# rusty-fast-solvers/rusty-compression

Hardware: AMD Instinct MI355X
Metric: GB/s + compressions/sec, 8192x8192 f64 rank-128 rSVD+ID (higher is better)
Workload: dtype f64

## Files before the change

rusty_compression_amd/csrc/kernels_qr.hip:

```cpp
#include "rc_common.hpp"
#include "rc_device.hpp"

namespace rc {

static __host__ __device__ inline int64_t cdiv(int64_t a, int64_t b) { return (a + b - 1) / b; }

template <typename T> struct Num;
template <> struct Num<double> {
    static __host__ __device__ inline double tol3z() { return 1.0536712127723509e-08; }
};
template <> struct Num<float> {
    static __host__ __device__ inline float tol3z() { return 2.44140625e-04f; }
};

template <typename T>
__device__ inline T wsum(T v) {
#pragma unroll
    for (int off = 32; off > 0; off >>= 1) v += __shfl_xor(v, off, 64);
    return v;
}

template <typename T, int TPC>
__device__ inline T group_sum(T v, T *sh ) {
    v = wsum(v);
// ... 258 lines not shown
        const int64_t rem_cols = n - j - 1;
        if (rem_cols <= 0) continue;
        const int64_t rem = m - j;
        const int64_t c64 = cdiv(rem, 64), c256 = cdiv(rem, 256);
#define RC_APPLY(TPC, MAXE)                                                                                       \
    hipLaunchKernelGGL((k_qr_apply<T, TPC, MAXE>), dim3((unsigned)cdiv(rem_cols, 256 / TPC)), dim3(256), 0,      \
                       c->stream, w, j, pv, jpvt, vn1, vn2, tau)
        if (c64 <= 2 && rem_cols >= 2048) {
            constexpr int CPW = 4;
            hipLaunchKernelGGL((k_qr_apply_short<T, CPW>), dim3((unsigned)cdiv(rem_cols, 4 * CPW)), dim3(256), 0, c->stream, w, j, pv, jpvt, vn1, vn2, tau);
        }
        else if (c64 <= 2) RC_APPLY(64, 2);
        else if (c64 <= 8) RC_APPLY(64, 8);
        else if (c256 <= 8) RC_APPLY(256, 8);
        else if (c256 <= 16) RC_APPLY(256, 16);
        else if (c256 <= 32) RC_APPLY(256, 32);
        else
            hipLaunchKernelGGL(k_qr_apply_general<T>, dim3((unsigned)rem_cols), dim3(256), 0, c->stream, w, j, pv, jpvt, vn1, vn2, tau);
#undef RC_APPLY
    }
}

template <typename T>
__global__ __launch_bounds__(256) void k_extract_r(Mat<T> w, const int64_t *jpvt, Mat<T> r) {
    const bool col_fast = (r.cs <= r.rs);
    const int64_t total = r.rows * r.cols;
    for (int64_t e = blockIdx.x * (int64_t)blockDim.x + threadIdx.x; e < total; e += (int64_t)gridDim.x * blockDim.x) {
        int64_t i, p;
        if (col_fast) { i = e / r.cols; p = e - i * r.cols; }
        else { p = e / r.rows; i = e - p * r.rows; }
        r.at(i, p) = (i <= p) ? w.p[jpvt[p] * w.cs + i] : (T)0;
    }
}
template <typename T>
void extract_r(rc_context *c, Mat<T> w, const int64_t *jpvt, Mat<T> r) {
    if (r.empty()) return;
    int grid = (int)std::min<int64_t>(cdiv(r.rows * r.cols, 256), 8192);
    hipLaunchKernelGGL(k_extract_r<T>, dim3(grid), dim3(256), 0, c->stream, w, jpvt, r);
}

template <typename T, int MAXE>
__global__ __launch_bounds__(256) void k_form_q(Mat<T> w, const int64_t *jpvt, const T *tau, int64_t k, Mat<T> qw) {
    __shared__ T sh[4];
    const int64_t m = w.rows;
    const int64_t cq = blockIdx.x;
    const int tid = threadIdx.x;
    T x[MAXE];
#pragma unroll
    for (int e = 0; e < MAXE; ++e) {
        int64_t i = tid + (int64_t)e * 256;
        x[e] = (i == cq) ? (T)1 : (T)0;
    }
    for (int64_t j = (cq < k - 1 ? cq : k - 1); j >= 0; --j) {
        const T tj = tau[j];
        if (tj == (T)0) continue;
// ... 22 lines not shown
}
template <typename T>
__global__ __launch_bounds__(256) void k_form_q_general(Mat<T> w, const int64_t *jpvt, const T *tau, int64_t k, Mat<T> qw) {
    __shared__ T sh[4];
    const int64_t m = w.rows;
    const int64_t cq = blockIdx.x;
    const int tid = threadIdx.x;
    T *x = qw.p + cq * qw.cs;
    for (int64_t i = tid; i < m; i += 256) x[i] = (i == cq) ? (T)1 : (T)0;
    for (int64_t j = (cq < k - 1 ? cq : k - 1); j >= 0; --j) {
        const T tj = tau[j];
        if (tj == (T)0) continue;
        const T *vcol = w.p + jpvt[j] * w.cs;
        const int64_t i0 = tid >= j ? tid : tid + ((j - tid + 255) / 256) * 256;
        T dot = 0;
        for (int64_t i = i0; i < m; i += 256) dot += ((i == j) ? (T)1 : vcol[i]) * x[i];
        dot = group_sum<T, 256>(dot, sh);
        const T f = tj * dot;
        for (int64_t i = i0; i < m; i += 256) x[i] -= f * ((i == j) ? (T)1 : vcol[i]);
    }
}

template <typename T, int NE>
__global__ __launch_bounds__(1024) void k_form_q_small(Mat<T> w, const int64_t *jpvt, const T *tau, int k, Mat<T> qw) {
    extern __shared__ __attribute__((aligned(16))) char smem_raw[];
    T *V = reinterpret_cast<T *>(smem_raw);
    T *tl = V + (size_t)k * 8 * NE;
    const int m = (int)w.rows;
    constexpr int LD = 8 * NE;
    for (int e = threadIdx.x; e < k * LD; e += blockDim.x) {
        const int j = e / LD, i = e - j * LD;
        V[e] = (i < j || i >= m) ? (T)0 : (i == j) ? (T)1 : w.p[jpvt[j] * w.cs + i];
    }
    for (int j = threadIdx.x; j < k; j += blockDim.x) tl[j] = tau[j];
    __syncthreads();
    const int l8 = threadIdx.x & 7, cq = threadIdx.x >> 3;
    if (cq >= qw.cols) return;
    T x[NE];
#pragma unroll
    for (int e = 0; e < NE; ++e) x[e] = (l8 + 8 * e == cq) ? (T)1 : (T)0;
    for (int j = cq < k - 1 ? cq : k - 1; j >= 0; --j) {
        const T tj = tl[j];
        if (tj == (T)0) continue;
        const T *vj = V + (size_t)j * LD + l8;
        T v[NE];
        T dot = 0;
#pragma unroll
        for (int e = 0; e < NE; ++e) {
            v[e] = vj[8 * e];
            dot = fma(v[e], x[e], dot);
        }
        dot = group_sum_dpp<8>(dot);
        const T f = tj * dot;
#pragma unroll
        for (int e = 0; e < NE; ++e) x[e] = fma(-f, v[e], x[e]);
    }
    T *out = qw.p + (int64_t)cq * qw.cs;
#pragma unroll
    for (int e = 0; e < NE; ++e) {
        const int i = l8 + 8 * e;
        if (i < m) out[i] = x[e];
    }
}

template <typename T>
__global__ __launch_bounds__(256) void k_extract_v(Mat<T> w, const int64_t *jpvt, Mat<T> vm) {
    const int64_t j = blockIdx.y;
    const T *col = w.p + jpvt[j] * w.cs;
    T *out = vm.p + j * vm.cs;
    for (int64_t i = blockIdx.x * 256 + threadIdx.x; i < vm.rows; i += (int64_t)gridDim.x * 256)
        out[i] = (i < j) ? (T)0 : (i == j) ? (T)1 : col[i];
}
template <typename T>
__global__ __launch_bounds__(1024) void k_build_t(Mat<T> sgram, const T *tau, Mat<T> tm) {
    extern __shared__ __attribute__((aligned(16))) char smem_raw[];
    T *svec = reinterpret_cast<T *>(smem_raw);
    T *trow = svec + tm.rows;
    const int k = (int)tm.rows;
    const int ld = k | 1;
    const int tid = threadIdx.x;
    for (int e = tid; e < k * ld; e += 1024) trow[e] = 0;
    __syncthreads();
    for (int j = 0; j < k; ++j) {
        for (int l = tid; l < j; l += 1024) svec[l] = sgram.at(l, j);
        __syncthreads();
// ... 105 lines not shown
#pragma unroll
                        for (int i2 = 0; i2 < ii; ++i2) acc[i2] -= tile[i2][ii] * acc[ii];
                    }
                }
            }
        }
        if (active) {
#pragma unroll
            for (int ii = 0; ii < NB; ++ii)
                if (r0 + ii < k) b.at(r0 + ii, col) = acc[ii];
        }
    }
}
template <typename T>
void trsm_upper(rc_context *c, Mat<T> t, Mat<T> b) {
    RC_REQUIRE(t.rows == t.cols && t.rows == b.rows, RC_INVALID_ARGUMENT, "trsm: shape mismatch");
    if (b.empty()) return;
    ProfScope ps(c, "op:trsm_upper k=%lld nrhs=%lld", (long long)t.rows, (long long)b.cols);
    hipLaunchKernelGGL(k_trsm_upper<T>, dim3((unsigned)cdiv(b.cols, 256)), dim3(256), 0, c->stream, t, b);
}

template <bool CHECKED> struct IdzCheck {};
template <> struct IdzCheck<true> { const int64_t *inv; int *health; };
template <typename T, bool FROM_R, bool CHECKED = false>
__global__ __launch_bounds__(256) void k_id_z(Mat<T> w, const int64_t *jpvt, int64_t k, Mat<T> z, IdzCheck<CHECKED> chk = {}) {
    static_assert(FROM_R || !CHECKED, "the ?geqp3-format variant only ever sees a jpvt the library wrote");
    constexpr int NB = 16;
    __shared__ T tile[NB][NB + 1];
    const int64_t n = w.cols;
    const int64_t p = blockIdx.x * (int64_t)blockDim.x + threadIdx.x;
    bool owns = p < n;
    if constexpr (CHECKED) {
        if (owns && chk.inv[p] < 0) {
            for (int64_t i = 0; i < k; ++i) z.at(i, p) = (T)0;
            atomicOr(chk.health, 32);
        }
        const int64_t e = owns ? jpvt[p] : -1;
        owns = (uint64_t)e < (uint64_t)n && chk.inv[e] == p;
    }
    const bool inside = owns;
    const int64_t dc = inside ? jpvt[p] : 0;
    const bool active = inside && p >= k;
    const T *bcol = FROM_R ? w.p + (inside ? p : 0) * w.cs : w.p + dc * w.cs;
    const int64_t brs = FROM_R ? w.rs : 1;
    const int64_t nblk = (k + NB - 1) / NB;
    const int ti = threadIdx.x / NB, tj = threadIdx.x % NB;
    if (inside && p < k)
        for (int64_t i = 0; i < k; ++i) z.at(i, dc) = (i == p) ? (T)1 : (T)0;
    for (int64_t bi = nblk - 1; bi >= 0; --bi) {
        const int64_t r0 = bi * NB;
        T acc[NB];
#pragma unroll
        for (int ii = 0; ii < NB; ++ii) acc[ii] = (active && r0 + ii < k) ? bcol[(r0 + ii) * brs] : (T)0;
        for (int64_t bj = nblk - 1; bj >= bi; --bj) {
            const int64_t c0 = bj * NB;
            __syncthreads();
            {
                const int64_t i = r0 + ti, l = c0 + tj;
                tile[ti][tj] = (i < k && l < k && i <= l) ? (FROM_R ? w.at(i, l) : w.p[jpvt[l] * w.cs + i]) : (T)0;
            }
            __syncthreads();
            if (bj > bi) {
                T x[NB];
#pragma unroll
                for (int jj = 0; jj < NB; ++jj) x[jj] = (active && c0 + jj < k) ? z.at(c0 + jj, dc) : (T)0;
#pragma unroll
                for (int jj = 0; jj < NB; ++jj)
#pragma unroll
                    for (int ii = 0; ii < NB; ++ii) acc[ii] -= tile[ii][jj] * x[jj];
            } else {
#pragma unroll
                for (int ii = NB - 1; ii >= 0; --ii) {
                    if (r0 + ii < k) {
                        acc[ii] /= tile[ii][ii];
#pragma unroll
                        for (int i2 = 0; i2 < ii; ++i2) acc[i2] -= tile[i2][ii] * acc[ii];
                    }
                }
            }
        }
        if (active) {
#pragma unroll
            for (int ii = 0; ii < NB; ++ii)
                if (r0 + ii < k) z.at(r0 + ii, dc) = acc[ii];
        }
    }
}
template <typename T>
void column_id_from_qrcp(rc_context *c, Mat<T> a, Mat<T> w, int64_t k, const int64_t *jpvt, Mat<T> cm, Mat<T> z) {
    RC_REQUIRE(w.rs == 1 && a.rows == w.rows && a.cols == w.cols && cm.rows == a.rows && cm.cols == k && z.rows == k && z.cols == a.cols && k <= std::min(a.rows, a.cols),
               RC_INVALID_ARGUMENT, "column_id_from_qrcp: shape mismatch");
    if (a.cols == 0 || k == 0) return;
    ProfScope ps(c, "op:column_id_from_qrcp %lldx%lld k=%lld", (long long)a.rows, (long long)a.cols, (long long)k);
    hipLaunchKernelGGL((k_id_z<T, false>), dim3((unsigned)cdiv(a.cols, 256)), dim3(256), 0, c->stream, w, jpvt, k, z);
    gather_cols(c, a, jpvt, cm);
}
template <typename T>
void id_z_from_r(rc_context *c, Mat<T> r, int64_t k, const int64_t *ind, Mat<T> z) {
    RC_REQUIRE(r.rows == k && z.rows == k && z.cols == r.cols && k <= r.cols, RC_INVALID_ARGUMENT, "id_z_from_r: shape mismatch");
    if (r.cols == 0 || k == 0) return;
    ProfScope ps(c, "op:id_z_from_r k=%lld n=%lld", (long long)k, (long long)r.cols);
    hipLaunchKernelGGL((k_id_z<T, true>), dim3((unsigned)cdiv(r.cols, 256)), dim3(256), 0, c->stream, r, ind, k, z);
}
template <typename T>
void id_z_from_r_checked(rc_context *c, Mat<T> r, int64_t k, const int64_t *ind, const int64_t *inv, Mat<T> z) {
    RC_REQUIRE(r.rows == k && z.rows == k && z.cols == r.cols && k <= r.cols, RC_INVALID_ARGUMENT, "id_z_from_r: shape mismatch");
    if (r.cols == 0 || k == 0) return;
    ProfScope ps(c, "op:id_z_from_r_checked k=%lld n=%lld", (long long)k, (long long)r.cols);
    hipLaunchKernelGGL((k_id_z<T, true, true>), dim3((unsigned)cdiv(r.cols, 256)), dim3(256), 0, c->stream, r, ind, k, z, IdzCheck<true>{inv, c->health_word()});
}

#define RC_INST(T)                                                                                         \
    template void column_id_from_qrcp<T>(rc_context *, Mat<T>, Mat<T>, int64_t, const int64_t *, Mat<T>, Mat<T>); \
    template void id_z_from_r<T>(rc_context *, Mat<T>, int64_t, const int64_t *, Mat<T>);                 \
    template void id_z_from_r_checked<T>(rc_context *, Mat<T>, int64_t, const int64_t *, const int64_t *, Mat<T>); \
    template void geqp3_inplace<T>(rc_context *, Mat<T>, int64_t, bool, int64_t *, T *, T *);             \
    template void extract_r<T>(rc_context *, Mat<T>, const int64_t *, Mat<T>);                             \
    template void form_q<T>(rc_context *, Mat<T>, const int64_t *, const T *, int64_t, Mat<T>);           \
    template void trsm_upper<T>(rc_context *, Mat<T>, Mat<T>);
RC_INST(double)
RC_INST(float)
#undef RC_INST

}

namespace rc {

template <typename T>
__global__ __launch_bounds__(256) void k_wq_init(Mat<T> qacc, Mat<T> rphys) {
    const int64_t tq = qacc.rows * qacc.cols, tr = rphys.rows * rphys.cols;
    for (int64_t e = blockIdx.x * (int64_t)blockDim.x + threadIdx.x; e < tq + tr; e += (int64_t)gridDim.x * blockDim.x) {
        if (e < tq) { int64_t i = e % qacc.rows, c2 = e / qacc.rows; qacc.p[c2 * qacc.cs + i] = (i == c2) ? (T)1 : (T)0; }
        else rphys.p[e - tq] = 0;
    }
}

template <typename T>
__global__ __launch_bounds__(1024) void k_wq_pivot(Mat<T> b, Mat<T> qacc, Mat<T> rphys, int64_t j, int64_t *jpvt, T *vn1, T *vn2, T *tau) {
    extern __shared__ __attribute__((aligned(16))) char smem_raw[];
    const int m = (int)b.rows;
// ... 248 lines not shown
```

rusty_compression_amd/csrc/kernels_tsqr.hip:

```cpp
#include "rc_common.hpp"
#include "rc_device.hpp"

namespace rc {

static __host__ __device__ inline int64_t cdiv(int64_t a, int64_t b) { return (a + b - 1) / b; }

template <typename T> struct TNum;
template <> struct TNum<double> {
    static __device__ inline double tol3z() { return 1.0536712127723509e-08; }
    static __device__ inline double tiny() { return 1e-300; }
};
template <> struct TNum<float> {
    static __device__ inline float tol3z() { return 2.44140625e-04f; }
    static __device__ inline float tiny() { return 1e-30f; }
};

template <typename T>
__device__ inline T wave_sum64(T v) {
#pragma unroll
    for (int off = 32; off > 0; off >>= 1) v += __shfl_xor(v, off, 64);
    return v;
}
template <typename T>
__device__ inline T row_sum16(T v) {
// ... 257 lines not shown
                    vn1[p] = vn * fast_sqrt_pos(temp);
                }
            }
        }
    }
}

template <typename T, int NE, int LPP, int E0>
__device__ __forceinline__ void qrcp_small_reflect(T (&x)[NE], const T *vcol, T tj, int j, int n, int ll) {
    T v[NE];
    T dot = 0;
#pragma unroll
    for (int e = E0; e < NE; ++e) {
        int i = ll + LPP * e;
        v[e] = 0;
        if (i < n && i >= j) { v[e] = (i == j) ? (T)1 : vcol[i]; dot = fma(v[e], x[e], dot); }
    }
    dot = group_sum_dpp<LPP>(dot);
    const T f = tj * dot;
#pragma unroll
    for (int e = E0; e < NE; ++e) x[e] -= f * v[e];
}

template <typename T, int NE, int NTHR>
__global__ __launch_bounds__(NTHR) void k_qrcp_small(Mat<T> rin, int kmax, int pivot, int64_t *jpvt_out, Mat<T> rout, Mat<T> q2) {
    constexpr int LPP = 8;
    constexpr int NGRP = NTHR / LPP;
    extern __shared__ __attribute__((aligned(16))) char smem_raw[];
    const int n = (int)rin.rows;
    const int ld = n | 1;
    T *A = reinterpret_cast<T *>(smem_raw);
    T *vn1 = A + (size_t)n * ld;
    T *vn2 = vn1 + n;
    T *tau = vn2 + n;
    int *jp = reinterpret_cast<int *>(tau + n);
    const int tid = threadIdx.x, lane = tid & 63;
    const int ll = tid % LPP, grp = tid / LPP;
    const bool safe = LPP * NE <= 3 * n;

    for (int e = tid; e < n * n; e += NTHR) {
        int i = e % n, cc = e / n;
        A[cc * ld + i] = rin.at(i, cc);
    }
    __syncthreads();
    for (int p = grp; p < n; p += NGRP) {
        T acc = 0;
        for (int i = ll; i < n; i += LPP) { T v = A[p * ld + i]; acc += v * v; }
        acc = group_sum_dpp<LPP>(acc);
// ... 35 lines not shown
                if (lane == 0) { tau[j] = (beta - alpha) * fast_rcp(beta); col[j] = beta; }
            }
        }
        __syncthreads();
        {
            const int rem = n - j;
            const T tj = tau[j];
            if (NE > 12 && rem > 8 * 12) qrcp_small_apply<T, NE, LPP>(A, ld, n, j, grp, ll, NGRP, jp, vn1, vn2, tj, pivot, safe);
            else if (NE > 8 && rem > 8 * 8) qrcp_small_apply<T, (NE > 12 ? 12 : NE), LPP>(A, ld, n, j, grp, ll, NGRP, jp, vn1, vn2, tj, pivot, safe);
            else if (NE > 4 && rem > 8 * 4) qrcp_small_apply<T, (NE > 8 ? 8 : NE), LPP>(A, ld, n, j, grp, ll, NGRP, jp, vn1, vn2, tj, pivot, safe);
            else qrcp_small_apply<T, (NE > 4 ? 4 : NE), LPP>(A, ld, n, j, grp, ll, NGRP, jp, vn1, vn2, tj, pivot, safe);
        }
        __syncthreads();
    }

    for (int p = tid; p < n; p += NTHR) jpvt_out[p] = jp[p];
    if (!rout.empty()) {
        const int64_t total = rout.rows * rout.cols;
        for (int64_t e = tid; e < total; e += NTHR) {
            int i = (int)(e / rout.cols), p = (int)(e % rout.cols);
            rout.at(i, p) = (i <= p) ? A[jp[p] * ld + i] : (T)0;
        }
    }
    if (!q2.empty()) {
        for (int cq = grp; cq < (int)q2.cols; cq += NGRP) {
            T x[NE];
#pragma unroll
            for (int e = 0; e < NE; ++e) x[e] = (ll + LPP * e == cq) ? (T)1 : (T)0;
            for (int j = (cq < kmax - 1 ? cq : kmax - 1); j >= 0; --j) {
                const T tj = tau[j];
                if (tj == (T)0) continue;
                const T *vcol = A + jp[j] * ld;
                const int e0 = j / LPP;
                if (NE > 12 && e0 >= 12) qrcp_small_reflect<T, NE, LPP, (NE > 12 ? 12 : 0)>(x, vcol, tj, j, n, ll);
                else if (NE > 8 && e0 >= 8) qrcp_small_reflect<T, NE, LPP, (NE > 8 ? 8 : 0)>(x, vcol, tj, j, n, ll);
                else if (NE > 4 && e0 >= 4) qrcp_small_reflect<T, NE, LPP, (NE > 4 ? 4 : 0)>(x, vcol, tj, j, n, ll);
                else qrcp_small_reflect<T, NE, LPP, 0>(x, vcol, tj, j, n, ll);
            }
#pragma unroll
            for (int e = 0; e < NE; ++e) {
                int i = ll + LPP * e;
                if (i < n) q2.at(i, cq) = x[e];
            }
        }
    }
}

template <typename T>
void qrcp_small(rc_context *c, Mat<T> rin, int64_t kmax, bool pivot, int64_t *jpvt, Mat<T> rout, Mat<T> q2) {
    const int64_t n = rin.rows;
    RC_REQUIRE(rin.rows == rin.cols, RC_INVALID_ARGUMENT, "qrcp_small: square input required");
    const size_t lds = ((size_t)n * (n | 1) + 3 * (size_t)n) * sizeof(T) + (size_t)n * sizeof(int) + 64;
    RC_REQUIRE(lds <= 160 * 1024 - 1024 && n <= 208, RC_INVALID_ARGUMENT, "qrcp_small: n = %lld does not fit LDS", (long long)n);
    ProfScope ps(c, "op:qrcp_small n=%lld k=%lld", (long long)n, (long long)kmax);
#define RC_QS(NE, NT_)                                                                                                 \
    do {                                                                                                               \
        auto kern = k_qrcp_small<T, NE, NT_>;                                                                          \
        static bool attr_set[64] = {};                                                                                 \
        if (!attr_set[c->device & 63]) {                                                                               \
            RC_HIP(hipFuncSetAttribute(reinterpret_cast<const void *>(kern), hipFuncAttributeMaxDynamicSharedMemorySize, 160 * 1024 - 1024)); \
            attr_set[c->device & 63] = true;                                                                           \
        }                                                                                                              \
        hipLaunchKernelGGL(kern, dim3(1), dim3(NT_), lds, c->stream, rin, (int)kmax, pivot ? 1 : 0, jpvt, rout, q2);   \
    } while (0)
    static const int wide = [] { const char *e = getenv("RC_QRCP_SMALL_1024"); return e ? atoi(e) : 1; }();
    if (n <= 64) RC_QS(8, 512);
    else if (n <= 144 && wide) RC_QS(18, 1024);
    else if (n <= 144) RC_QS(18, 512);
    else RC_QS(26, 512);
#undef RC_QS
}

template <typename T>
__global__ __launch_bounds__(1024) void k_householder_signs(Mat<T> q, T *d) {
    extern __shared__ __attribute__((aligned(16))) char smem_raw[];
    const int k = (int)q.cols;
    const int ld = k | 1;
    T *W = reinterpret_cast<T *>(smem_raw);
    const int tid = threadIdx.x;
    for (int e = tid; e < k * k; e += 1024) {
        int i = e % k, cc = e / k;
        W[i * ld + cc] = q.at(i, cc);
    }
    __syncthreads();
    const int ti = tid >> 5, tc = tid & 31;
    for (int j = 0; j < k; ++j) {
        const T s = W[j * ld + j];
        const T dj = (s > (T)0) ? (T)-1 : (T)1;
// ... 99 lines not shown
```

rusty_compression_amd/csrc/rc_api.hip:

```cpp
#include "rc_common.hpp"

#include <unistd.h>

#include <atomic>
#include <chrono>

#include <algorithm>
#include <cmath>

using namespace rc;

static constexpr size_t kAlign = 256;

void rc_context::retire_arena() {
    if (arena) {
        if (live_graphs > 0) retired.push_back(arena);
        else (void)hipFree(arena);
    }
    arena = nullptr;
    arena_size = 0;
}

void rc_context::swap_arena() {
    std::swap(arena, aux_arena.base);
// ... 361 lines not shown
    int64_t *ident = c->alloc<int64_t>((size_t)k);
    iota_i64(c, ident, k);
    Mat<T> w = a.sub(0, m, 0, k);
    if (!(w.rs == 1 && w.cs >= m)) {
        Mat<T> wc = tmp_colmajor<T>(c, m, k);
        copy_mat(c, w, wc);
        w = wc;
    }
    if (q.rs == 1 && q.cs >= q.rows) {
        form_q(c, w, ident, tau, k, q);
    } else {
        Mat<T> qw = tmp_colmajor<T>(c, m, k);
        form_q(c, w, ident, tau, k, qw);
        copy_mat(c, qw, q);
    }
}

static int tsqr_fold() {
    static const int fold = [] { const char *e = getenv("RC_TSQR_FOLD"); return e ? atoi(e) : 1; }();
    return fold;
}

template <typename T>
void svd_finish(rc_context *c, bool transposed, bool factored, Mat<T> qw, Mat<T> q1, Mat<T> r2i, Mat<T> uc, Mat<T> vc, const T *s, Mat<T> u, Mat<T> vt) {
    const int64_t r = uc.rows;
    complete_left_basis(c, uc, s);
    Mat<T> small;
    if (factored) {
        small = tmp_colmajor<T>(c, r, r);
        gemm<T>(c, 1, r2i, transposed ? vc : uc, 0, small);
    }
    if (!transposed) {
        if (factored) gemm<T>(c, 1, q1, small, 0, u);
        else gemm<T>(c, 1, qw, uc, 0, u);
        copy_mat(c, vc.t(), vt);
    } else {
        copy_mat(c, uc, u);
        if (factored) gemm<T>(c, 1, small.t(), q1.t(), 0, vt);
        else gemm<T>(c, 1, vc.t(), qw.t(), 0, vt);
    }
}

template <typename T>
void svd_core(rc_context *c, Mat<T> wt, bool transposed, Mat<T> u, T *s, Mat<T> vt) {
    const int64_t M = wt.rows, r = wt.cols;
    ArenaMark mark(c);
    Mat<T> core = tmp_colmajor<T>(c, r, r);
    Mat<T> qw, q1, r2i;
    bool done = false;
    const int fold = tsqr_fold();
    if (c->opt_tsqr && tsqr_supported<T>(M, r)) {
        if (fold) {
            q1 = rowmajor(c->alloc<T>((size_t)M * even_ld(r)), M, r, even_ld(r));
            r2i = rowmajor(c->alloc<T>((size_t)r * even_ld(r)), r, r, even_ld(r));
            done = run_certified(c, [&](int *flag) { tsqr_cholqr2_factored<T>(c, wt, q1, r2i, transposed ? core.t() : core, flag); });
        } else {
            qw = tmp_colmajor<T>(c, M, r);
            done = run_certified(c, [&](int *flag) { tsqr_cholqr2<T>(c, wt, qw, transposed ? core.t() : core, flag); });
        }
    }
// ... 7 lines not shown
        extract_r(c, wt, jp, transposed ? core.t() : core);
        form_q(c, wt, jp, tau, r, qw);
    }
    Mat<T> vwork = tmp_colmajor<T>(c, r, r), uc = tmp_colmajor<T>(c, r, r), vc = tmp_colmajor<T>(c, r, r);
    jacobi_svd(c, core, vwork, uc, s, vc);
    svd_finish(c, transposed, factored, qw, q1, r2i, uc, vc, s, u, vt);
}

template <typename T>
void compute_svd(rc_context *c, Mat<T> a, Mat<T> u, T *s, Mat<T> vt) {
    const int64_t m = a.rows, n = a.cols, r = std::min(m, n);
    RC_REQUIRE(u.rows == m && u.cols == r && vt.rows == r && vt.cols == n, RC_INVALID_ARGUMENT,
               "compute_svd: a %lld x %lld needs u %lld x %lld, vt %lld x %lld", (long long)m, (long long)n, (long long)m,
               (long long)r, (long long)r, (long long)n);
    if (r == 0) return;
    ArenaMark mark(c);
    const bool transposed = m < n;
    Mat<T> src = transposed ? a.t() : a;
    Mat<T> wt = tmp_colmajor<T>(c, src.rows, src.cols);
    copy_mat(c, src, wt);
    svd_core(c, wt, transposed, u, s, vt);
}

template <typename T>
void qr_column_id(rc_context *c, Mat<T> q, Mat<T> r, const int64_t *ind, Mat<T> cm, Mat<T> z, bool own_ind) {
    const int64_t m = q.rows, k = q.cols, n = r.cols;
    RC_REQUIRE(r.rows == k && cm.rows == m && cm.cols == k && z.rows == k && z.cols == n, RC_INVALID_ARGUMENT,
               "column_id: q %lld x %lld, r %lld x %lld, c %lld x %lld, z %lld x %lld", (long long)m, (long long)k,
               (long long)r.rows, (long long)n, (long long)cm.rows, (long long)cm.cols, (long long)z.rows, (long long)z.cols);
    RC_REQUIRE(k <= n, RC_INVALID_ARGUMENT, "column_id: rank exceeds the number of columns");
    if (n == 0) return;
    ArenaMark mark(c);
    static const int fused = [] { const char *e = getenv("RC_ID_FUSED"); return e ? atoi(e) : 1; }();
    if (fused && k < n) {
        if (own_ind) {
            id_z_from_r(c, r, k, ind, z);
        } else {
            int64_t *inv = c->alloc<int64_t>((size_t)n);
            invert_perm(c, ind, n, inv);
            id_z_from_r_checked(c, r, k, ind, inv, z);
        }
        gemm<T>(c, 1, q, r.sub(0, k, 0, k), 0, cm);
        return;
    }
    int64_t *inv = c->alloc<int64_t>((size_t)n);
    invert_perm(c, ind, n, inv);
    Mat<T> zt = tmp_rowmajor<T>(c, k, n);
    if (k == n) {
        gemm<T>(c, 1, q, r, 0, cm);
        fill_identity(c, zt);
    } else {
        fill_identity(c, zt.sub(0, k, 0, k));
        copy_mat(c, r.sub(0, k, k, n - k), zt.sub(0, k, k, n - k));
        trsm_upper(c, r.sub(0, k, 0, k), zt.sub(0, k, k, n - k));
        gemm<T>(c, 1, q, r.sub(0, k, 0, k), 0, cm);
    }
    gather_cols(c, zt, inv, z);
// ... 271 lines not shown
        ProfScope ps(c, "stage:project B=Q^H A");
        a.project(c, range, b);
    }
    rsvd_id_consumers(c, range, b, o);
}

template <typename T>
bool fused_consumers_qualify(rc_context *c, int64_t k, int64_t n) {
    return c->opt_fused_consumers && c->opt_wide_coop && c->opt_tsqr && tsqr_fold() && c->lanes_in_flight() < 8 && tsqr_supported<T>(n, k) &&
           wide_coop_jacobi_supported<T>(k, n, c->device);
}

template <typename T>
bool rsvd_id_consumers_fused(rc_context *c, Mat<T> range, Mat<T> b, const rc_rsvd_id_out &o) {
    const int64_t m = range.rows, k = b.rows, n = b.cols;
    ArenaMark mark(c);
    Mat<T> core = tmp_colmajor<T>(c, k, k);
    Mat<T> q1 = rowmajor(c->alloc<T>((size_t)n * even_ld(k)), n, k, even_ld(k));
    Mat<T> r2i = rowmajor(c->alloc<T>((size_t)k * even_ld(k)), k, k, even_ld(k));
    {
        ProfScope ps(c, "stage:tall QR of B^T");
        if (!run_certified(c, [&](int *flag) { tsqr_cholqr2_factored<T>(c, b.t(), q1, r2i, core.t(), flag); })) return false;
    }
    Mat<T> uc = tmp_colmajor<T>(c, k, k), vc = tmp_colmajor<T>(c, k, k);
    Mat<T> qb = tmp_colmajor<T>(c, k, k);
    Mat<T> r = o.qr_r.data ? from_c<T>(o.qr_r) : tmp_rowmajor<T>(c, k, n);
    int64_t *ind = o.qr_ind ? o.qr_ind : c->alloc<int64_t>((size_t)n);
    T *tau = c->alloc<T>((size_t)k);
    Mat<T> wf = tmp_colmajor<T>(c, k, n);
    T *s = static_cast<T *>(o.s);
    bool qr_done;
    {
        ProfScope ps(c, "stage:qrcp of B | svd of the core");
        qr_done = run_certified(c, [&](int *flag) { geqp3_wide_coop_jacobi<T>(c, b, wf, k, ind, tau, flag, core, uc, s, vc); });
    }
    {
        ProfScope ps(c, "stage:qrcp of B + column_id");
        if (qr_done) {
            extract_r(c, wf, ind, r);
            form_q(c, wf, ind, tau, k, qb);
        } else {
            qrcp_core(c, b, k, true, qb, r, ind);
        }
        Mat<T> q = o.qr_q.data ? from_c<T>(o.qr_q) : tmp_colmajor<T>(c, m, k);
        gemm<T>(c, 1, range, qb, 0, q);
        if (o.id_c.data || o.id_z.data) qr_column_id(c, q, r, ind, from_c<T>(o.id_c), from_c<T>(o.id_z), true);
    }
    {
        ProfScope ps(c, "stage:svd of B + U=Q Ub");
        Mat<T> ub = tmp_colmajor<T>(c, k, k);
        svd_finish(c, true, true, Mat<T>(), q1, r2i, uc, vc, s, ub, from_c<T>(o.vt));
        gemm<T>(c, 1, range, ub, 0, from_c<T>(o.u));
    }
    return true;
}

template <typename T>
void rsvd_id_consumers(rc_context *c, Mat<T> range, Mat<T> b, const rc_rsvd_id_out &o) {
    const int64_t m = range.rows, k = b.rows, n = b.cols;
    const bool want_id = o.id_c.data || o.id_z.data || o.qr_q.data || o.qr_r.data || o.qr_ind;
    const bool want_svd = o.u.data || o.s || o.vt.data;
    if (want_svd) RC_REQUIRE(o.u.data && o.s && o.vt.data, RC_INVALID_ARGUMENT, "rsvd_id: u, s, vt must be given together");
    if (want_id && want_svd && !c->opt_fork && fused_consumers_qualify<T>(c, k, n)) {
        RC_REQUIRE(!(o.id_c.data || o.id_z.data) || (o.id_c.data && o.id_z.data), RC_INVALID_ARGUMENT, "rsvd_id: id_c and id_z must be given together");
        if (rsvd_id_consumers_fused(c, range, b, o)) return;
    }
    Mat<T> wq;
    if (want_id && want_svd && c->opt_fork) {
        wq = tmp_colmajor<T>(c, k, n);
        copy_mat(c, b, wq);
    }
    Fork fork(c, want_svd && want_id);
    if (want_id) {
        ProfScope ps(c, "stage:qrcp of B + column_id");
// ... 977 lines not shown
```

rusty_compression_amd/csrc/rc_common.hpp:

```cpp
#pragma once

#include <hip/hip_runtime.h>

#include <cstdarg>
#include <cstdint>
#include <cstdio>
#include <cstring>
#include <map>
#include <string>
#include <vector>

#include "../../include/rusty_compression_amd.h"

namespace rc {

template <typename T>
struct Mat {
    T *p = nullptr;
    int64_t rows = 0, cols = 0, rs = 0, cs = 0;

    __host__ __device__ Mat() {}
    __host__ __device__ Mat(T *p_, int64_t r, int64_t c, int64_t rs_, int64_t cs_) : p(p_), rows(r), cols(c), rs(rs_), cs(cs_) {}
    __host__ __device__ inline T &at(int64_t i, int64_t j) const { return p[i * rs + j * cs]; }
    __host__ __device__ Mat<T> sub(int64_t r0, int64_t nr, int64_t c0, int64_t nc) const {
// ... 226 lines not shown
template <typename T> bool qrb_finish(BlockedQrcpJob<T> *job);
template <typename T> void qrb_form_q(BlockedQrcpJob<T> *job, Mat<T> q);
template <typename T> void qrb_end(BlockedQrcpJob<T> *job);
struct QrbState;
template <typename T> bool qrb_optimistic_possible(BlockedQrcpJob<T> *job);
template <typename T> bool qrb_issue_all_optimistic(BlockedQrcpJob<T> *job);
template <typename T> bool qrb_verify_optimistic(BlockedQrcpJob<T> *job);
template <typename T> bool qrb_verify_optimistic(const QrbState *host_log, const std::vector<int> &nbp_log, bool broken);
template <typename T> void qrb_optimistic_log(BlockedQrcpJob<T> *job, const QrbState **log, std::vector<int> *nbp_log, bool *broken);
template <typename T> void qrb_keep_t(BlockedQrcpJob<T> *job, bool keep);
template <typename T> bool wide_lazy_supported(int64_t m, int64_t n);
template <typename T> void geqp3_wide_lazy(rc_context *c, Mat<T> b, int64_t kmax, int64_t *jpvt, Mat<T> q, Mat<T> r);
template <typename T> bool wide_coop_supported(int64_t m, int64_t n, int device);
template <typename T> void geqp3_wide_coop(rc_context *c, Mat<T> w, Mat<T> wf, int64_t kmax, int64_t *jpvt, T *tau, int *flag);
template <typename T> bool wide_coop_jacobi_supported(int64_t m, int64_t n, int device);
template <typename T>
void geqp3_wide_coop_jacobi(rc_context *c, Mat<T> w, Mat<T> wf, int64_t kmax, int64_t *jpvt, T *tau, int *flag, Mat<T> core, Mat<T> uc, T *s, Mat<T> vc);
void coop_prepare(int device);
unsigned *coop_semaphore_of(int device);
unsigned coop_budget_units(int device);
void coop_gate_launch(rc_context *c, unsigned need, unsigned *sync, unsigned long long *hdr, int hdr_words, const int *proceed = nullptr, unsigned *clr = nullptr,
                      int clr_words = 0);
template <typename T> void extract_r(rc_context *c, Mat<T> w, const int64_t *jpvt, Mat<T> r);
template <typename T> void form_q(rc_context *c, Mat<T> w, const int64_t *jpvt, const T *tau, int64_t k, Mat<T> qw);
template <typename T> void trsm_upper(rc_context *c, Mat<T> t, Mat<T> b);
template <typename T> bool tsqr_supported(int64_t m, int64_t n);
template <typename T> void tsqr_cholqr2(rc_context *c, Mat<T> y, Mat<T> q, Mat<T> r, int *flag);
template <typename T> void tsqr_cholqr2_factored(rc_context *c, Mat<T> y, Mat<T> q1, Mat<T> r2i, Mat<T> r, int *flag);
template <typename T> void qrcp_small(rc_context *c, Mat<T> rin, int64_t kmax, bool pivot, int64_t *jpvt, Mat<T> rout, Mat<T> q2);
template <typename T> void householder_sign_fix(rc_context *c, Mat<T> q, Mat<T> r);
template <typename T> void qrcp_tall_fast(rc_context *c, Mat<T> y, int64_t k, bool pivot, Mat<T> q, Mat<T> r, int64_t *ind, int *flag);
template <typename T> void jacobi_svd(rc_context *c, Mat<T> g, Mat<T> vwork, Mat<T> uc, T *s, Mat<T> vc);

}
```

Measured before the change: 728.7.

## Fuse QRCP tail kernels into one launch and split small-QRCP Q formation

Merges extract_r, form_q_small and the ID Z solve into a single heterogeneous kernel whose workgroups are partitioned by role. C is then computed as Q·R[:, :k] instead of going through the general column-ID path. Separately, qrcp_small now writes a shared-memory image to global memory so a multi-workgroup kernel can form Q2 in parallel rather than on one block. The copy of the core U is also elided by computing it in place, and several copy loops are unrolled to keep more loads in flight. The cost is an extra global round-trip for the image, more code paths, and a shape-restricted fused path (64<k<=128).

Result: faster. 745.3 (median of 6 runs) (+2.3%).

```diff
diff --git a/rusty_compression_amd/csrc/kernels_qr.hip b/rusty_compression_amd/csrc/kernels_qr.hip
--- a/rusty_compression_amd/csrc/kernels_qr.hip
+++ b/rusty_compression_amd/csrc/kernels_qr.hip
@@ -304,15 +304,31 @@
 }
 
 template <typename T>
-__global__ __launch_bounds__(256) void k_extract_r(Mat<T> w, const int64_t *jpvt, Mat<T> r) {
+__device__ __forceinline__ void extract_r_body(Mat<T> w, const int64_t *jpvt, Mat<T> r, int64_t wg, int64_t nwg, int tid, int nthr) {
     const bool col_fast = (r.cs <= r.rs);
     const int64_t total = r.rows * r.cols;
-    for (int64_t e = blockIdx.x * (int64_t)blockDim.x + threadIdx.x; e < total; e += (int64_t)gridDim.x * blockDim.x) {
-        int64_t i, p;
-        if (col_fast) { i = e / r.cols; p = e - i * r.cols; }
-        else { p = e / r.rows; i = e - p * r.rows; }
-        r.at(i, p) = (i <= p) ? w.p[jpvt[p] * w.cs + i] : (T)0;
-    }
+    constexpr int U = 4;
+    const int64_t stride = nwg * nthr;
+    for (int64_t e0 = wg * (int64_t)nthr + tid; e0 < total; e0 += stride * U) {
+        T val[U];
+        T *dst[U];
+#pragma unroll
+        for (int u = 0; u < U; ++u) {
+            const int64_t e = e0 + u * stride < total ? e0 + u * stride : e0;
+            int64_t i, p;
+            if (col_fast) { i = e / r.cols; p = e - i * r.cols; }
+            else { p = e / r.rows; i = e - p * r.rows; }
+            dst[u] = &r.at(i, p);
+            val[u] = (i <= p) ? w.p[jpvt[p] * w.cs + i] : (T)0;
+        }
+#pragma unroll
+        for (int u = 0; u < U; ++u)
+            if (e0 + u * stride < total) *dst[u] = val[u];
+    }
+}
+template <typename T>
+__global__ __launch_bounds__(256) void k_extract_r(Mat<T> w, const int64_t *jpvt, Mat<T> r) {
+    extract_r_body<T>(w, jpvt, r, blockIdx.x, gridDim.x, threadIdx.x, blockDim.x);
 }
 template <typename T>
 void extract_r(rc_context *c, Mat<T> w, const int64_t *jpvt, Mat<T> r) {
@@ -381,19 +397,28 @@
 }
 
 template <typename T, int NE>
-__global__ __launch_bounds__(1024) void k_form_q_small(Mat<T> w, const int64_t *jpvt, const T *tau, int k, Mat<T> qw) {
-    extern __shared__ __attribute__((aligned(16))) char smem_raw[];
+__device__ __forceinline__ void form_q_small_body(Mat<T> w, const int64_t *jpvt, const T *tau, int k, Mat<T> qw, char *smem_raw, int wg, int tid, int nthr) {
     T *V = reinterpret_cast<T *>(smem_raw);
     T *tl = V + (size_t)k * 8 * NE;
     const int m = (int)w.rows;
     constexpr int LD = 8 * NE;
-    for (int e = threadIdx.x; e < k * LD; e += blockDim.x) {
-        const int j = e / LD, i = e - j * LD;
-        V[e] = (i < j || i >= m) ? (T)0 : (i == j) ? (T)1 : w.p[jpvt[j] * w.cs + i];
-    }
-    for (int j = threadIdx.x; j < k; j += blockDim.x) tl[j] = tau[j];
+    const int kst = min(k, (wg + 1) * (nthr >> 3));
+    constexpr int U = 8;
+    for (int e0 = tid; e0 < kst * LD; e0 += nthr * U) {
+        T val[U];
+#pragma unroll
+        for (int u = 0; u < U; ++u) {
+            const int e = e0 + u * nthr;
+            const int j = min(e / LD, kst - 1), i = e & (LD - 1);
+            val[u] = (i < j || i >= m) ? (T)0 : (i == j) ? (T)1 : w.p[jpvt[j] * w.cs + i];
+        }
+#pragma unroll
+        for (int u = 0; u < U; ++u)
+            if (e0 + u * nthr < kst * LD) V[e0 + u * nthr] = val[u];
+    }
+    for (int j = tid; j < k; j += nthr) tl[j] = tau[j];
     __syncthreads();
-    const int l8 = threadIdx.x & 7, cq = threadIdx.x >> 3;
+    const int l8 = tid & 7, cq = wg * (nthr >> 3) + (tid >> 3);
     if (cq >= qw.cols) return;
     T x[NE];
 #pragma unroll
@@ -420,6 +445,11 @@
         const int i = l8 + 8 * e;
         if (i < m) out[i] = x[e];
     }
+}
+template <typename T, int NE>
+__global__ __launch_bounds__(1024) void k_form_q_small(Mat<T> w, const int64_t *jpvt, const T *tau, int k, Mat<T> qw) {
+    extern __shared__ __attribute__((aligned(16))) char smem_raw[];
+    form_q_small_body<T, NE>(w, jpvt, tau, k, qw, smem_raw, 0, threadIdx.x, blockDim.x);
 }
 
 template <typename T>
@@ -571,13 +601,14 @@
 
 template <bool CHECKED> struct IdzCheck {};
 template <> struct IdzCheck<true> { const int64_t *inv; int *health; };
-template <typename T, bool FROM_R, bool CHECKED = false>
-__global__ __launch_bounds__(256) void k_id_z(Mat<T> w, const int64_t *jpvt, int64_t k, Mat<T> z, IdzCheck<CHECKED> chk = {}) {
+constexpr int kIdzNB = 16;
+template <typename T, bool FROM_R, bool CHECKED>
+__device__ __forceinline__ void id_z_body(Mat<T> w, const int64_t *jpvt, const int64_t *jtri, int64_t k, Mat<T> z, IdzCheck<CHECKED> chk, T (*tile)[kIdzNB + 1], int64_t wg,
+                                          int tid, int nthr) {
     static_assert(FROM_R || !CHECKED, "the ?geqp3-format variant only ever sees a jpvt the library wrote");
-    constexpr int NB = 16;
-    __shared__ T tile[NB][NB + 1];
+    constexpr int NB = kIdzNB;
     const int64_t n = w.cols;
-    const int64_t p = blockIdx.x * (int64_t)blockDim.x + threadIdx.x;
+    const int64_t p = wg * (int64_t)nthr + tid;
     bool owns = p < n;
     if constexpr (CHECKED) {
         if (owns && chk.inv[p] < 0) {
@@ -593,7 +624,7 @@
     const T *bcol = FROM_R ? w.p + (inside ? p : 0) * w.cs : w.p + dc * w.cs;
     const int64_t brs = FROM_R ? w.rs : 1;
     const int64_t nblk = (k + NB - 1) / NB;
-    const int ti = threadIdx.x / NB, tj = threadIdx.x % NB;
+    const int ti = tid / NB, tj = tid % NB;
     if (inside && p < k)
         for (int64_t i = 0; i < k; ++i) z.at(i, dc) = (i == p) ? (T)1 : (T)0;
     for (int64_t bi = nblk - 1; bi >= 0; --bi) {
@@ -606,7 +637,7 @@
             __syncthreads();
             {
                 const int64_t i = r0 + ti, l = c0 + tj;
-                tile[ti][tj] = (i < k && l < k && i <= l) ? (FROM_R ? w.at(i, l) : w.p[jpvt[l] * w.cs + i]) : (T)0;
+                tile[ti][tj] = (i < k && l < k && i <= l) ? (FROM_R ? w.at(i, l) : w.p[jtri[l] * w.cs + i]) : (T)0;
             }
             __syncthreads();
             if (bj > bi) {
@@ -634,6 +665,45 @@
                 if (r0 + ii < k) z.at(r0 + ii, dc) = acc[ii];
         }
     }
+}
+template <typename T, bool FROM_R, bool CHECKED = false>
+__global__ __launch_bounds__(256) void k_id_z(Mat<T> w, const int64_t *jpvt, int64_t k, Mat<T> z, IdzCheck<CHECKED> chk = {}) {
+    __shared__ T tile[kIdzNB][kIdzNB + 1];
+    id_z_body<T, FROM_R, CHECKED>(w, jpvt, jpvt, k, z, chk, tile, blockIdx.x, threadIdx.x, blockDim.x);
+}
+
+template <typename T, int NE>
+__global__ __launch_bounds__(256) void k_rsvd_id_tails(Mat<T> w, const int64_t *jpvt, const T *tau, int k, Mat<T> z, Mat<T> qw, Mat<T> r, int nz, int nq) {
+    extern __shared__ __attribute__((aligned(16))) char smem_raw[];
+    __shared__ T tile[kIdzNB][kIdzNB + 1];
+    __shared__ int64_t jtri[8 * NE];
+    const int wg = (int)blockIdx.x, tid = (int)threadIdx.x;
+    if (wg < nz) {
+        for (int j = tid; j < k; j += 256) jtri[j] = jpvt[j];
+        __syncthreads();
+        id_z_body<T, false, false>(w, jpvt, jtri, k, z, IdzCheck<false>{}, tile, wg, tid, 256);
+    }
+    else if (wg < nz + nq) form_q_small_body<T, NE>(w, jpvt, tau, k, qw, smem_raw, wg - nz, tid, 256);
+    else extract_r_body<T>(w, jpvt, r, wg - nz - nq, (int64_t)gridDim.x - nz - nq, tid, 256);
+}
+template <typename T>
+void rsvd_id_tails(rc_context *c, Mat<T> wf, const int64_t *jpvt, const T *tau, Mat<T> qb, Mat<T> r, Mat<T> z) {
+    const int64_t k = wf.rows, n = wf.cols;
+    RC_REQUIRE(wf.rs == 1 && qb.rs == 1 && qb.rows == k && qb.cols == k && r.rows == k && r.cols == n && k > 64 && k <= 8 * 16 && k < n &&
+                   (z.empty() || (z.rows == k && z.cols == n)),
+               RC_INVALID_ARGUMENT, "rsvd_id_tails: shape mismatch");
+    constexpr int NE = 16, CPW = 256 / 8;
+    const int nz = z.empty() ? 0 : (int)cdiv(n, 256), nq = (int)cdiv(qb.cols, CPW);
+    const int nr = (int)std::min<int64_t>(cdiv(k * n, 256), 192);
+    const size_t lds = ((size_t)k * 8 * NE + (size_t)k) * sizeof(T);
+    ProfScope ps(c, "op:rsvd_id_tails k=%lld n=%lld wgs=%d+%d+%d", (long long)k, (long long)n, nz, nq, nr);
+    auto kern = k_rsvd_id_tails<T, NE>;
+    static bool attr_set[64] = {};
+    if (!attr_set[c->device & 63]) {
+        RC_HIP(hipFuncSetAttribute(reinterpret_cast<const void *>(kern), hipFuncAttributeMaxDynamicSharedMemorySize, 160 * 1024 - 4096));
+        attr_set[c->device & 63] = true;
+    }
+    hipLaunchKernelGGL(kern, dim3((unsigned)(nz + nq + nr)), dim3(256), lds, c->stream, wf, jpvt, tau, (int)k, z, qb, r, nz, nq);
 }
 template <typename T>
 void column_id_from_qrcp(rc_context *c, Mat<T> a, Mat<T> w, int64_t k, const int64_t *jpvt, Mat<T> cm, Mat<T> z) {
@@ -665,6 +735,7 @@
     template void id_z_from_r_checked<T>(rc_context *, Mat<T>, int64_t, const int64_t *, const int64_t *, Mat<T>); \
     template void geqp3_inplace<T>(rc_context *, Mat<T>, int64_t, bool, int64_t *, T *, T *);             \
     template void extract_r<T>(rc_context *, Mat<T>, const int64_t *, Mat<T>);                             \
+    template void rsvd_id_tails<T>(rc_context *, Mat<T>, const int64_t *, const T *, Mat<T>, Mat<T>, Mat<T>); \
     template void form_q<T>(rc_context *, Mat<T>, const int64_t *, const T *, int64_t, Mat<T>);           \
     template void trsm_upper<T>(rc_context *, Mat<T>, Mat<T>);
 RC_INST(double)
diff --git a/rusty_compression_amd/csrc/kernels_tsqr.hip b/rusty_compression_amd/csrc/kernels_tsqr.hip
--- a/rusty_compression_amd/csrc/kernels_tsqr.hip
+++ b/rusty_compression_amd/csrc/kernels_tsqr.hip
@@ -303,8 +303,69 @@
     for (int e = E0; e < NE; ++e) x[e] -= f * v[e];
 }
 
-template <typename T, int NE, int NTHR>
-__global__ __launch_bounds__(NTHR) void k_qrcp_small(Mat<T> rin, int kmax, int pivot, int64_t *jpvt_out, Mat<T> rout, Mat<T> q2) {
+template <typename T, int NE, int LPP, int E0>
+__device__ __forceinline__ void qrcp_small_reflect_flat(T (&x)[NE], const T *vcol, T tj, int j, int n, int ll) {
+    T v[NE];
+    bool on[NE];
+#pragma unroll
+    for (int e = E0; e < NE; ++e) {
+        const int i = ll + LPP * e;
+        on[e] = i < n && i >= j;
+        v[e] = vcol[on[e] ? i : j];
+    }
+#pragma unroll
+    for (int e = E0; e < NE; ++e) asm volatile("" : "+v"(v[e]));
+#pragma unroll
+    for (int e = E0; e < NE; ++e) v[e] = on[e] ? ((ll + LPP * e == j) ? (T)1 : v[e]) : (T)0;
+    T dot = 0;
+#pragma unroll
+    for (int e = E0; e < NE; ++e) dot = on[e] ? fma(v[e], x[e], dot) : dot;
+    dot = group_sum_dpp<LPP>(dot);
+    const T f = tj * dot;
+#pragma unroll
+    for (int e = E0; e < NE; ++e) x[e] -= f * v[e];
+}
+
+template <typename T, int NE, int LPP, bool FLAT = false>
+__device__ __forceinline__ void qrcp_small_q2_column(const T *A, int ld, int n, int kmax, const T *tau, const int *jp, int cq, int ll, Mat<T> q2) {
+    T x[NE];
+#pragma unroll
+    for (int e = 0; e < NE; ++e) x[e] = (ll + LPP * e == cq) ? (T)1 : (T)0;
+    const int j0 = cq < kmax - 1 ? cq : kmax - 1;
+    T tnext = tau[j0 > 0 ? j0 : 0];
+    int pnext = jp[j0 > 0 ? j0 : 0];
+    for (int j = j0; j >= 0; --j) {
+        const T tj = FLAT ? tnext : tau[j];
+        if (tj == (T)0) {
+            if constexpr (FLAT) { const int jn = j > 0 ? j - 1 : 0; tnext = tau[jn]; pnext = jp[jn]; }
+            continue;
+        }
+        const T *vcol = A + (FLAT ? pnext : jp[j]) * ld;
+        const int e0 = j / LPP;
+        if constexpr (FLAT) {
+            const int jn = j > 0 ? j - 1 : 0;
+            tnext = tau[jn];
+            pnext = jp[jn];
+            if (NE > 12 && e0 >= 12) qrcp_small_reflect_flat<T, NE, LPP, (NE > 12 ? 12 : 0)>(x, vcol, tj, j, n, ll);
+            else if (NE > 8 && e0 >= 8) qrcp_small_reflect_flat<T, NE, LPP, (NE > 8 ? 8 : 0)>(x, vcol, tj, j, n, ll);
+            else if (NE > 4 && e0 >= 4) qrcp_small_reflect_flat<T, NE, LPP, (NE > 4 ? 4 : 0)>(x, vcol, tj, j, n, ll);
+            else qrcp_small_reflect_flat<T, NE, LPP, 0>(x, vcol, tj, j, n, ll);
+            continue;
+        }
+        if (NE > 12 && e0 >= 12) qrcp_small_reflect<T, NE, LPP, (NE > 12 ? 12 : 0)>(x, vcol, tj, j, n, ll);
+        else if (NE > 8 && e0 >= 8) qrcp_small_reflect<T, NE, LPP, (NE > 8 ? 8 : 0)>(x, vcol, tj, j, n, ll);
+        else if (NE > 4 && e0 >= 4) qrcp_small_reflect<T, NE, LPP, (NE > 4 ? 4 : 0)>(x, vcol, tj, j, n, ll);
+        else qrcp_small_reflect<T, NE, LPP, 0>(x, vcol, tj, j, n, ll);
+    }
+#pragma unroll
+    for (int e = 0; e < NE; ++e) {
+        int i = ll + LPP * e;
+        if (i < n) q2.at(i, cq) = x[e];
+    }
+}
+
+template <typename T, int NE, int NTHR, bool IMG = false>
+__global__ __launch_bounds__(NTHR) void k_qrcp_small(Mat<T> rin, int kmax, int pivot, int64_t *jpvt_out, Mat<T> rout, Mat<T> q2, T *img = nullptr) {
     constexpr int LPP = 8;
     constexpr int NGRP = NTHR / LPP;
     extern __shared__ __attribute__((aligned(16))) char smem_raw[];
@@ -386,28 +447,43 @@
             rout.at(i, p) = (i <= p) ? A[jp[p] * ld + i] : (T)0;
         }
     }
+    if constexpr (IMG) {
+        const int nt = n * ld + 3 * n;
+        for (int e = tid; e < nt; e += NTHR) img[e] = A[e];
+        int *ijp = reinterpret_cast<int *>(img + nt);
+        for (int p = tid; p < n; p += NTHR) ijp[p] = jp[p];
+        return;
+    }
     if (!q2.empty()) {
-        for (int cq = grp; cq < (int)q2.cols; cq += NGRP) {
-            T x[NE];
-#pragma unroll
-            for (int e = 0; e < NE; ++e) x[e] = (ll + LPP * e == cq) ? (T)1 : (T)0;
-            for (int j = (cq < kmax - 1 ? cq : kmax - 1); j >= 0; --j) {
-                const T tj = tau[j];
-                if (tj == (T)0) continue;
-                const T *vcol = A + jp[j] * ld;
-                const int e0 = j / LPP;
-                if (NE > 12 && e0 >= 12) qrcp_small_reflect<T, NE, LPP, (NE > 12 ? 12 : 0)>(x, vcol, tj, j, n, ll);
-                else if (NE > 8 && e0 >= 8) qrcp_small_reflect<T, NE, LPP, (NE > 8 ? 8 : 0)>(x, vcol, tj, j, n, ll);
-                else if (NE > 4 && e0 >= 4) qrcp_small_reflect<T, NE, LPP, (NE > 4 ? 4 : 0)>(x, vcol, tj, j, n, ll);
-                else qrcp_small_reflect<T, NE, LPP, 0>(x, vcol, tj, j, n, ll);
-            }
-#pragma unroll
-            for (int e = 0; e < NE; ++e) {
-                int i = ll + LPP * e;
-                if (i < n) q2.at(i, cq) = x[e];
-            }
-        }
-    }
+        for (int cq = grp; cq < (int)q2.cols; cq += NGRP) qrcp_small_q2_column<T, NE, LPP>(A, ld, n, kmax, tau, jp, cq, ll, q2);
+    }
+}
+
+template <typename T, int NE>
+__global__ __launch_bounds__(1024) void k_qrcp_small_q2(const T *img, int n, int kmax, Mat<T> q2, int cpw) {
+    constexpr int LPP = 8;
+    extern __shared__ __attribute__((aligned(16))) char smem_raw[];
+    const int ld = n | 1;
+    T *A = reinterpret_cast<T *>(smem_raw);
+    T *tau = A + (size_t)n * ld + 2 * n;
+    int *jp = reinterpret_cast<int *>(tau + n);
+    const int tid = threadIdx.x;
+    const int nt = n * ld + 3 * n;
+    constexpr int U = 8;
+    for (int e0 = tid; e0 < nt; e0 += 1024 * U) {
+        T val[U];
+#pragma unroll
+        for (int u = 0; u < U; ++u) val[u] = img[min(e0 + 1024 * u, nt - 1)];
+#pragma unroll
+        for (int u = 0; u < U; ++u)
+            if (e0 + 1024 * u < nt) A[e0 + 1024 * u] = val[u];
+    }
+    const int *ijp = reinterpret_cast<const int *>(img + nt);
+    for (int p = tid; p < n; p += 1024) jp[p] = ijp[p];
+    __syncthreads();
+    const int ll = tid % LPP, grp = tid / LPP;
+    const int cq = (int)blockIdx.x * cpw + grp;
+    if (grp < cpw && cq < (int)q2.cols) qrcp_small_q2_column<T, NE, LPP, true>(A, ld, n, kmax, tau, jp, cq, ll, q2);
 }
 
 template <typename T>
@@ -425,9 +501,28 @@
             RC_HIP(hipFuncSetAttribute(reinterpret_cast<const void *>(kern), hipFuncAttributeMaxDynamicSharedMemorySize, 160 * 1024 - 1024)); \
             attr_set[c->device & 63] = true;                                                                           \
         }                                                                                                              \
-        hipLaunchKernelGGL(kern, dim3(1), dim3(NT_), lds, c->stream, rin, (int)kmax, pivot ? 1 : 0, jpvt, rout, q2);   \
+        hipLaunchKernelGGL(kern, dim3(1), dim3(NT_), lds, c->stream, rin, (int)kmax, pivot ? 1 : 0, jpvt, rout, q2, (T *)nullptr); \
     } while (0)
     static const int wide = [] { const char *e = getenv("RC_QRCP_SMALL_1024"); return e ? atoi(e) : 1; }();
+    static const int q2_wgs = [] { const char *e = getenv("RC_QRCP_Q2_WGS"); return e ? std::min(std::max(atoi(e), 0), 64) : 8; }();
+    if (n > 64 && n <= 144 && wide && q2_wgs > 0 && !q2.empty() && c->lanes_in_flight() < 8) {
+        ArenaMark mark(c);
+        const size_t nt = (size_t)n * (n | 1) + 3 * (size_t)n;
+        T *img = c->alloc<T>(nt + (size_t)n);
+        auto kf = k_qrcp_small<T, 18, 1024, true>;
+        auto kq = k_qrcp_small_q2<T, 18>;
+        static bool attr_set[64] = {};
+        if (!attr_set[c->device & 63]) {
+            RC_HIP(hipFuncSetAttribute(reinterpret_cast<const void *>(kf), hipFuncAttributeMaxDynamicSharedMemorySize, 160 * 1024 - 1024));
+            RC_HIP(hipFuncSetAttribute(reinterpret_cast<const void *>(kq), hipFuncAttributeMaxDynamicSharedMemorySize, 160 * 1024 - 1024));
+            attr_set[c->device & 63] = true;
+        }
+        hipLaunchKernelGGL(kf, dim3(1), dim3(1024), lds, c->stream, rin, (int)kmax, pivot ? 1 : 0, jpvt, rout, q2, img);
+        const int cpw = (int)std::min<int64_t>(cdiv(cdiv(q2.cols, q2_wgs), 8) * 8, 128);
+        ProfScope pq(c, "op:qrcp_small_q2 n=%lld cols=%lld wgs=%d", (long long)n, (long long)q2.cols, (int)cdiv(q2.cols, cpw));
+        hipLaunchKernelGGL(kq, dim3((unsigned)cdiv(q2.cols, cpw)), dim3(1024), lds, c->stream, (const T *)img, (int)n, (int)kmax, q2, cpw);
+        return;
+    }
     if (n <= 64) RC_QS(8, 512);
     else if (n <= 144 && wide) RC_QS(18, 1024);
     else if (n <= 144) RC_QS(18, 512);
diff --git a/rusty_compression_amd/csrc/rc_api.hip b/rusty_compression_amd/csrc/rc_api.hip
--- a/rusty_compression_amd/csrc/rc_api.hip
+++ b/rusty_compression_amd/csrc/rc_api.hip
@@ -407,7 +407,8 @@
 }
 
 template <typename T>
-void svd_finish(rc_context *c, bool transposed, bool factored, Mat<T> qw, Mat<T> q1, Mat<T> r2i, Mat<T> uc, Mat<T> vc, const T *s, Mat<T> u, Mat<T> vt) {
+void svd_finish(rc_context *c, bool transposed, bool factored, Mat<T> qw, Mat<T> q1, Mat<T> r2i, Mat<T> uc, Mat<T> vc, const T *s, Mat<T> u, Mat<T> vt,
+                bool u_in_place = false) {
     const int64_t r = uc.rows;
     complete_left_basis(c, uc, s);
     Mat<T> small;
@@ -420,7 +421,7 @@
         else gemm<T>(c, 1, qw, uc, 0, u);
         copy_mat(c, vc.t(), vt);
     } else {
-        copy_mat(c, uc, u);
+        if (!u_in_place) copy_mat(c, uc, u);
         if (factored) gemm<T>(c, 1, small.t(), q1.t(), 0, vt);
         else gemm<T>(c, 1, vc.t(), qw.t(), 0, vt);
     }
@@ -474,6 +475,11 @@
     svd_core(c, wt, transposed, u, s, vt);
 }
 
+static int id_fused() {
+    static const int fused = [] { const char *e = getenv("RC_ID_FUSED"); return e ? atoi(e) : 1; }();
+    return fused;
+}
+
 template <typename T>
 void qr_column_id(rc_context *c, Mat<T> q, Mat<T> r, const int64_t *ind, Mat<T> cm, Mat<T> z, bool own_ind) {
     const int64_t m = q.rows, k = q.cols, n = r.cols;
@@ -483,8 +489,7 @@
     RC_REQUIRE(k <= n, RC_INVALID_ARGUMENT, "column_id: rank exceeds the number of columns");
     if (n == 0) return;
     ArenaMark mark(c);
-    static const int fused = [] { const char *e = getenv("RC_ID_FUSED"); return e ? atoi(e) : 1; }();
-    if (fused && k < n) {
+    if (id_fused() && k < n) {
         if (own_ind) {
             id_z_from_r(c, r, k, ind, z);
         } else {
@@ -802,7 +807,7 @@
         ProfScope ps(c, "stage:tall QR of B^T");
         if (!run_certified(c, [&](int *flag) { tsqr_cholqr2_factored<T>(c, b.t(), q1, r2i, core.t(), flag); })) return false;
     }
-    Mat<T> uc = tmp_colmajor<T>(c, k, k), vc = tmp_colmajor<T>(c, k, k);
+    Mat<T> ub = tmp_colmajor<T>(c, k, k), vc = tmp_colmajor<T>(c, k, k);
     Mat<T> qb = tmp_colmajor<T>(c, k, k);
     Mat<T> r = o.qr_r.data ? from_c<T>(o.qr_r) : tmp_rowmajor<T>(c, k, n);
     int64_t *ind = o.qr_ind ? o.qr_ind : c->alloc<int64_t>((size_t)n);
@@ -812,11 +817,19 @@
     bool qr_done;
     {
         ProfScope ps(c, "stage:qrcp of B | svd of the core");
-        qr_done = run_certified(c, [&](int *flag) { geqp3_wide_coop_jacobi<T>(c, b, wf, k, ind, tau, flag, core, uc, s, vc); });
+        qr_done = run_certified(c, [&](int *flag) { geqp3_wide_coop_jacobi<T>(c, b, wf, k, ind, tau, flag, core, ub, s, vc); });
     }
     {
         ProfScope ps(c, "stage:qrcp of B + column_id");
-        if (qr_done) {
+        const bool want_cz = o.id_c.data || o.id_z.data;
+        Mat<T> cm = from_c<T>(o.id_c), z = from_c<T>(o.id_z);
+        const bool tails = qr_done && k < n && id_fused();
+        if (tails) {
+            if (want_cz)
+                RC_REQUIRE(cm.rows == m && cm.cols == k && z.rows == k && z.cols == n, RC_INVALID_ARGUMENT, "column_id: c %lld x %lld, z %lld x %lld",
+                           (long long)cm.rows, (long long)cm.cols, (long long)z.rows, (long long)z.cols);
+            rsvd_id_tails(c, wf, ind, tau, qb, r, want_cz ? z : Mat<T>());
+        } else if (qr_done) {
             extract_r(c, wf, ind, r);
             form_q(c, wf, ind, tau, k, qb);
         } else {
@@ -824,12 +837,12 @@
         }
         Mat<T> q = o.qr_q.data ? from_c<T>(o.qr_q) : tmp_colmajor<T>(c, m, k);
         gemm<T>(c, 1, range, qb, 0, q);
-        if (o.id_c.data || o.id_z.data) qr_column_id(c, q, r, ind, from_c<T>(o.id_c), from_c<T>(o.id_z), true);
+        if (want_cz && tails) gemm<T>(c, 1, q, r.sub(0, k, 0, k), 0, cm);
+        else if (want_cz) qr_column_id(c, q, r, ind, cm, z, true);
     }
     {
         ProfScope ps(c, "stage:svd of B + U=Q Ub");
-        Mat<T> ub = tmp_colmajor<T>(c, k, k);
-        svd_finish(c, true, true, Mat<T>(), q1, r2i, uc, vc, s, ub, from_c<T>(o.vt));
+        svd_finish(c, true, true, Mat<T>(), q1, r2i, ub, vc, s, ub, from_c<T>(o.vt), true);
         gemm<T>(c, 1, range, ub, 0, from_c<T>(o.u));
     }
     return true;
diff --git a/rusty_compression_amd/csrc/rc_common.hpp b/rusty_compression_amd/csrc/rc_common.hpp
--- a/rusty_compression_amd/csrc/rc_common.hpp
+++ b/rusty_compression_amd/csrc/rc_common.hpp
@@ -272,6 +272,7 @@
 void coop_gate_launch(rc_context *c, unsigned need, unsigned *sync, unsigned long long *hdr, int hdr_words, const int *proceed = nullptr, unsigned *clr = nullptr,
                       int clr_words = 0);
 template <typename T> void extract_r(rc_context *c, Mat<T> w, const int64_t *jpvt, Mat<T> r);
+template <typename T> void rsvd_id_tails(rc_context *c, Mat<T> wf, const int64_t *jpvt, const T *tau, Mat<T> qb, Mat<T> r, Mat<T> z);
 template <typename T> void form_q(rc_context *c, Mat<T> w, const int64_t *jpvt, const T *tau, int64_t k, Mat<T> qw);
 template <typename T> void trsm_upper(rc_context *c, Mat<T> t, Mat<T> b);
 template <typename T> bool tsqr_supported(int64_t m, int64_t n);
```
